# ViennaRNA/RNAcode

Hardware: AMD Instinct MI355X
Metric: alignment-columns x samples scored /sec (higher is better)
Workload: dtype f32; 1 GPU; synthetic MAF 10000 blocks x 120 cols x 6 seqs, n=1000 (BASELINE configs[2]/[3]); exchange=none, fit_exp_mode=fused

## Files before the change

rnacode_amd/csrc/rc_null_kernel.h:

```cpp
#pragma once
#include <hip/hip_runtime.h>

#include <type_traits>
#include <utility>

#include "rc_device.h"
#include "rc_launch.h"

namespace rc {


template <bool SEM> __device__ __forceinline__ float ref_max(float x, float y) {
  if constexpr (SEM) return x > y ? x : y;
  else return fmaxf(x, y);
}
template <bool SEM> __device__ __forceinline__ float ref_max3(float x, float y, float z) { return ref_max<SEM>(ref_max<SEM>(x, y), z); }

template <bool SEM = false>
__device__ __forceinline__ void pair_step(int zc, float sig, float Delta, float Omega, float omega,
                                          float &s0, float &s1, float &s2) {
  if (zc == 0) {
    s0 = s0 + sig;
    s1 = s1 + omega;
    s2 = s2 + omega;
// ... 29 lines not shown

__device__ __forceinline__ void native_scan_rows(const float *rows, int aLo, int aHi, int sites, int s, int f, float tieThr, ScanState &st, int &n,
                                                 DevHss *out, int hssCap, int lane) {
  for (int a = aLo; a < aHi; a++) {
    for (int j0 = a; j0 < sites; j0 += kWave) {
      const int j = j0 + lane;
      const float v = (j < sites) ? rows[static_cast<size_t>(a - aLo) * sites + j] : 0.0f;
      const bool last = (a == sites - 1) && (j == sites - 1);
      unsigned long long m = __ballot((j < sites) && (v > 0.0f || last));
      while (m) {
        const int t = __builtin_ctzll(m);
        m &= m - 1ull;
        const int jj = j0 + t;
        const float vt = __int_as_float(__builtin_amdgcn_readlane(__float_as_int(v), t));
        scan_step(st, vt, a, jj, (a == sites - 1) && (jj == sites - 1), tieThr, [&](const ScanState &e) {
          if (out && lane == 0 && n < hssCap) out[n] = DevHss{s, f, e.ss, e.se, e.cm};
          n++;
        });
      }
    }
  }
}

__device__ __forceinline__ uint32_t codon_flip(uint32_t c) { return ((c & 3u) << 4) | (c & 12u) | ((c >> 4) & 3u); }


template <int K> struct KReg { float s0, s1, s2; int lut; };
template <typename Seq> struct KRegs;
template <int... K> struct KRegs<std::integer_sequence<int, K...>> : KReg<K>... {
  template <int I> __device__ __forceinline__ KReg<I> &at() { return static_cast<KReg<I> &>(*this); }
};
template <int NK, typename F, int... K>
__device__ __forceinline__ void static_for_impl(F &&f, std::integer_sequence<int, K...>) {
  (f(std::integral_constant<int, K>{}), ...);
}
template <int NK, typename F> __device__ __forceinline__ void static_for(F &&f) {
  static_for_impl<NK>(static_cast<F &&>(f), std::make_integer_sequence<int, NK>{});
}

template <int NK, bool EXACT> __device__ __forceinline__ float div_by_nk(float x, float nkf) {
  if constexpr ((NK & (NK - 1)) == 0) {
    return x * (1.0f / static_cast<float>(NK));
  } else if constexpr (EXACT) {
    return x / nkf;
  } else {
    constexpr float y = 1.0f / static_cast<float>(NK);
    const float q0 = x * y;
    const float r = __builtin_fmaf(-static_cast<float>(NK), q0, x);
    return __builtin_fmaf(r, y, q0);
  }
}

struct SampleScan {
  float cm;
  float Q;
  uint32_t se;
  uint32_t len;
};
__device__ __forceinline__ void sample_scan_row_begin(SampleScan &st, float &best, uint32_t a) {
  const bool done = (st.cm > 0.0f) & (st.se < a);
  best = (done & (st.len >= 2u) & (st.cm > best)) ? st.cm : best;
  st.cm = done ? 0.0f : st.cm;
  st.len = done ? 0u : st.len;
  st.Q = static_cast<float>(2u * (st.len + a));
}
__device__ __forceinline__ void sample_scan_step(SampleScan &st, float v, float j2, float negTieThr) {
  const float d = v - st.cm;
  const bool upd = (v > st.cm) | ((v > 0.0f) & (d > negTieThr) & (st.Q <= j2));
  st.cm = upd ? v : st.cm;
  st.Q = upd ? j2 : st.Q;
}
__device__ __forceinline__ void sample_scan_row_end(SampleScan &st, uint32_t a) {
  const uint32_t q = static_cast<uint32_t>(st.Q);
  const bool inrow = (q & 1u) != 0u;
  const uint32_t j = q >> 1;
  st.se = inrow ? j : st.se;
  st.len = inrow ? j - a : st.len;
}
__device__ __forceinline__ void sample_scan_last(const SampleScan &st, float &best) {
  best = ((st.len >= 2u) & (st.cm > best)) ? st.cm : best;
}

struct DeepFetch {};

template <int NK, bool LDSC, bool EXACT, bool DUAL, int MODE = 0>
__device__ __forceinline__ void null_body(const NullArgs &A, const uint8_t *__restrict__ blob,
                                          const DevBlock *__restrict__ dblocks, const int *__restrict__ classBlocks,
                                          const uint32_t *__restrict__ flags, const uint32_t *__restrict__ Ustream, const uint8_t *__restrict__ pairTab,
                                          uint32_t *__restrict__ scratch, float *__restrict__ maxima) {
  constexpr int N = NK + 1;
  constexpr int CPW = 5;
  constexpr int NCW = (NK + CPW - 1) / CPW;
  constexpr bool kTableLookups = !LDSC && !EXACT;
  constexpr int kTableWords = kTableLookups ? NK * kWave : 0;
  constexpr int LB = code_tail_bytes(NK);
  constexpr int PSW = code_pos_words(NK);
  using TailT = std::conditional_t<LB == 1, uint8_t, std::conditional_t<LB == 2, uint16_t, uint32_t>>;
  constexpr int ZW = (NK + 31) / 32;
  using Regs = KRegs<std::make_integer_sequence<int, NK>>;
  static_assert(!DUAL || (!EXACT && NK <= kDualRowsMaxNK), "two rows per pass: fast division, few sequences");
  static_assert(!(LDSC && EXACT), "the EXACT instantiation uses no LDS");
  constexpr bool ROWS = MODE == 1, SIM = MODE == 2;
#ifndef RC_DEEP_FETCH_MAX_NK
#define RC_DEEP_FETCH_MAX_NK 31
#endif
  constexpr bool kDeep = !LDSC && !EXACT && !DUAL && MODE == 0 && NK <= RC_DEEP_FETCH_MAX_NK;
  static_assert(MODE == 0 || (!LDSC && !EXACT && !DUAL), "rows split over workgroups: the one-row kernel that reads its codes from L2");
  extern __shared__ uint32_t lds_codes[];

  const int lane = threadIdx.x;
  unsigned int xcc;
  asm volatile("s_getreg_b32 %0, hwreg(HW_REG_XCC_ID)" : "=s"(xcc));
  const int home = static_cast<int>(xcc & 7u);
  const int rowParts = ROWS ? A.rowParts : 1;
  const int parts = SIM ? A.simParts : A.comboSplit ? 6 * rowParts : 1;
  const int nBlocks = A.nBlocksPtr ? *A.nBlocksPtr : A.nClassBlocks;
  const bool stealing = A.steal != nullptr && !A.comboSplit;
  constexpr int kStealHdr = 16;
  auto claim_part = [&](int slot) -> int {
    unsigned int v = 0;
    if (lane == 0) v = atomicAdd(A.steal + kStealHdr + slot, 1u);
    v = static_cast<unsigned int>(__builtin_amdgcn_readfirstlane(static_cast<int>(v)));
    return (v >= 1u && v <= 6u) ? static_cast<int>(v) - 1 : 6;
  };
  auto steal_word = [&](size_t at) -> unsigned int { return __hip_atomic_load(A.steal + at, __ATOMIC_RELAXED, __HIP_MEMORY_SCOPE_AGENT); };
  int helpCursor = 0;
  bool helping = false;
  for (int qi = 0;;) {
    int bi, grp, onlyCombo = -1, firstCombo = 0, rowPart = 0, itemIndex = 0;
    bool shared = false;
    int slot = static_cast<int>(blockIdx.x);
    if (!helping) {
      if (qi >= 8) {
        if (!stealing) break;
        helping = true;
        continue;
      }
      const int q = (home + qi) & 7;
      const int g0 = A.gLo + ((q - A.gLo) & 7);
      const int gq = g0 < A.gHi ? ((A.gHi - 1 - g0) >> 3) + 1 : 0;
      const int perBlock = gq * parts;
      const int nq = nBlocks * perBlock;
      int t = nq;
      if (nq > 0) {
        if (lane == 0) t = static_cast<int>(atomicAdd((SIM ? A.simCounter : A.workCounter) + q, 1u));
        t = __builtin_amdgcn_readfirstlane(t);
      }
      if (t >= nq) { qi++; continue; }
      bi = classBlocks[t / perBlock];
      if (A.skipMask && (flags[bi] & A.skipMask)) continue;
      const int sub = t % perBlock;
      grp = g0 + 8 * (sub / parts);
      onlyCombo = A.comboSplit ? (sub % parts) / rowParts : -1;
      if constexpr (MODE != 0) { rowPart = SIM ? sub % parts : (sub % parts) % rowParts; itemIndex = (t / perBlock) * (A.gHi - A.gLo) + (grp - A.gLo); }
      if constexpr (MODE != 0) slot = itemIndex;
      if (stealing && nq - t <= static_cast<int>(gridDim.x >> 3) + 16) {
        shared = true;
        if (lane == 0) atomicAdd(A.steal + 1, 1u);
      }
    } else {
      const size_t G = gridDim.x;
      const int np = __builtin_amdgcn_readfirstlane(static_cast<int>(steal_word(0)));
      int victim = -1;
      while (helpCursor < np) {
        const int i = helpCursor + lane;
        const unsigned int ent = i < np ? steal_word(kStealHdr + 3 * G + i) : 0u;
// ... 168 lines not shown
    if constexpr (SIM) continue;
    if (!helping && shared) {
      const size_t G = gridDim.x;
      if (lane == 0) {
        __hip_atomic_store(A.steal + kStealHdr + G + 2 * blockIdx.x, static_cast<unsigned int>(bi), __ATOMIC_RELAXED, __HIP_MEMORY_SCOPE_AGENT);
        __hip_atomic_store(A.steal + kStealHdr + G + 2 * blockIdx.x + 1, static_cast<unsigned int>(grp), __ATOMIC_RELAXED, __HIP_MEMORY_SCOPE_AGENT);
      }
      __builtin_amdgcn_fence(__ATOMIC_RELEASE, "agent");
      __builtin_amdgcn_s_waitcnt(0);
      if (lane == 0) {
        atomicExch(A.steal + kStealHdr + blockIdx.x, 1u);
        const unsigned int idx = atomicAdd(A.steal, 1u);
        __hip_atomic_store(A.steal + kStealHdr + 3 * G + idx, (blockIdx.x + 1u) | (static_cast<unsigned int>(home) << 24), __ATOMIC_RELAXED, __HIP_MEMORY_SCOPE_AGENT);
        atomicSub(A.steal + 1, 1u);
      }
      firstCombo = claim_part(slot);
    }

    float best = -1.0f;
    unsigned long long statCells = 0, statNoPos = 0, statPosLanes = 0, statPristine = 0, statEvent = 0, statTail = 0;
    float omega_v, Delta_v = 0.0f;
    asm volatile("v_mov_b32 %0, %1" : "=v"(omega_v) : "s"(omega));
    float rcpNk_v = 0.0f, negNk_v = 0.0f;
    if constexpr (!EXACT && (NK & (NK - 1)) != 0) {
      asm volatile("v_mov_b32 %0, %1" : "=v"(rcpNk_v) : "s"(1.0f / static_cast<float>(NK)));
      asm volatile("v_mov_b32 %0, %1" : "=v"(negNk_v) : "s"(-static_cast<float>(NK)));
    }
    if constexpr (EXACT) asm volatile("v_mov_b32 %0, %1" : "=v"(Delta_v) : "s"(Delta));
    if (!kProfiling || !(A.debugSkip & 1)) {
      Regs R;
      int curS = -1;
      for (int c = onlyCombo >= 0 ? onlyCombo : firstCombo; c < 6; c = onlyCombo >= 0 ? 6 : (shared ? claim_part(slot) : c + 1)) {
        const int s = c >= 3 ? 1 : 0, f = c - 3 * s;
        if (s != curS) {
          static_for<NK>([&](auto kc) {
            constexpr int k = decltype(kc)::value;
            R.template at<k>().lut = __float_as_int(lut[(s * NK + k) * kLutSize + lane]);
            if constexpr (kTableLookups) lds_codes[k * kWave + lane] = static_cast<uint32_t>(R.template at<k>().lut);
          });
          curS = s;
        }
        const int sites = (L - f) / 3;
        if (sites <= 0) continue;
        const uint32_t *__restrict__ sbase = cod + static_cast<size_t>(s * L1 + 3 + f) * PSW;
        constexpr int kSiteWords = 3 * PSW;
        auto word_at = [&](int j, int x) -> uint32_t {
          const uint32_t *p = sbase + static_cast<size_t>(j) * kSiteWords;
          if (x < NCW - 1) return p[x * kWave + lane];
          return static_cast<uint32_t>(reinterpret_cast<const TailT *>(p + (NCW - 1) * kWave)[lane]);
        };
        const unsigned long long *__restrict__ zbase = zw + static_cast<size_t>(s * L1 + 3 + f) * ZW;
        const unsigned long long *__restrict__ zany = zmask + static_cast<size_t>(s * 3 + f) * zmWords;
        int jc = sites;
        constexpr int kCacheSiteBytes = PSW * 4;
        if constexpr (LDSC) {
          for (int idx = 0; idx < sites * NCW; idx++) lds_codes[idx * kWave + lane] = word_at(idx / NCW, idx % NCW);
          __builtin_amdgcn_s_waitcnt(0);
        } else if constexpr (!EXACT) {
          jc = sites - (A.cacheSites < sites ? A.cacheSites : sites);
          for (int j = jc; j < sites; j++) {
            uint32_t *dst = lds_codes + kTableWords + (j - jc) * PSW;
#pragma unroll
            for (int x = 0; x < NCW - 1; x++) dst[x * kWave + lane] = word_at(j, x);
            reinterpret_cast<TailT *>(dst + (NCW - 1) * kWave)[lane] = static_cast<TailT>(word_at(j, NCW - 1));
          }
          __builtin_amdgcn_s_waitcnt(0);
        }
        const uint32_t ldsBase = static_cast<uint32_t>(reinterpret_cast<uintptr_t>(lds_codes + kTableWords));
        const uint32_t ldsLane = ldsBase + static_cast<uint32_t>(lane) * 4u;
        const uint32_t ldsTail = ldsBase + (NCW - 1) * kWave * 4u + static_cast<uint32_t>(lane) * LB;
        const uint32_t laneOff = static_cast<uint32_t>(lane) * 4u, laneTail = static_cast<uint32_t>(lane) * LB;
        [[maybe_unused]] const uint8_t *ldsBytesAll = reinterpret_cast<const uint8_t *>(lds_codes + kTableWords) - ldsBase;
        auto fetch_staged = [&](uint32_t (&w)[NCW], int j) {
          const uint32_t at = ldsLane + static_cast<uint32_t>(j) * (NCW * kWave * 4u);
#pragma unroll
          for (int x = 0; x < NCW; x++) {
#ifdef RC_PLAIN_FETCH
            w[x] = *reinterpret_cast<const uint32_t *>(ldsBytesAll + at + x * kWave * 4);
#else
            asm volatile("ds_read_b32 %0, %1 offset:%2" : "=v"(w[x]) : "v"(at), "n"(x * kWave * 4));
#endif
          }
        };
        auto fetch_cached = [&](uint32_t (&w)[NCW], int j) {
          const uint32_t off = static_cast<uint32_t>(j - jc) * kCacheSiteBytes;
#ifdef RC_PLAIN_FETCH
          if constexpr (NCW > 1) {
#pragma unroll
            for (int x = 0; x < NCW - 1; x++) w[x] = *reinterpret_cast<const uint32_t *>(ldsBytesAll + ldsLane + off + x * kWave * 4);
          }
          w[NCW - 1] = static_cast<uint32_t>(*reinterpret_cast<const TailT *>(ldsBytesAll + ldsTail + off));
#else
          if constexpr (NCW > 1) {
            const uint32_t at = ldsLane + off;
#pragma unroll
            for (int x = 0; x < NCW - 1; x++) asm volatile("ds_read_b32 %0, %1 offset:%2" : "=v"(w[x]) : "v"(at), "n"(x * kWave * 4));
          }
          const uint32_t att = ldsTail + off;
          if constexpr (LB == 1) asm volatile("ds_read_u8 %0, %1" : "=v"(w[NCW - 1]) : "v"(att));
          else if constexpr (LB == 2) asm volatile("ds_read_u16 %0, %1" : "=v"(w[NCW - 1]) : "v"(att));
          else asm volatile("ds_read_b32 %0, %1" : "=v"(w[NCW - 1]) : "v"(att));
#endif
        };
        auto fetch_global = [&](uint32_t (&w)[NCW], const uint32_t *p) {
          const uint32_t lo = laneOff + 0u, lt = laneTail + 0u;
#ifdef RC_PLAIN_FETCH
          const uint8_t *pb = reinterpret_cast<const uint8_t *>(p);
#pragma unroll
          for (int x = 0; x < NCW - 1; x++) w[x] = *reinterpret_cast<const uint32_t *>(pb + lo + x * kWave * 4);
          w[NCW - 1] = static_cast<uint32_t>(*reinterpret_cast<const TailT *>(pb + lt + (NCW - 1) * kWave * 4));
          return;
#endif
#pragma unroll
          for (int x = 0; x < NCW - 1; x++) asm volatile("global_load_dword %0, %1, %2 offset:%3" : "=v"(w[x]) : "v"(lo), "s"(p), "n"(x * kWave * 4));
          if constexpr (LB == 1) asm volatile("global_load_ubyte %0, %1, %2 offset:%3" : "=v"(w[NCW - 1]) : "v"(lt), "s"(p), "n"((NCW - 1) * kWave * 4));
          else if constexpr (LB == 2) asm volatile("global_load_ushort %0, %1, %2 offset:%3" : "=v"(w[NCW - 1]) : "v"(lt), "s"(p), "n"((NCW - 1) * kWave * 4));
          else asm volatile("global_load_dword %0, %1, %2 offset:%3" : "=v"(w[NCW - 1]) : "v"(lt), "s"(p), "n"((NCW - 1) * kWave * 4));
        };
        auto load_words = [&](int j, uint32_t (&w)[NCW]) {
          if constexpr (LDSC) {
#pragma unroll
            for (int x = 0; x < NCW; x++) w[x] = lds_codes[(j * NCW + x) * kWave + lane];
          } else if constexpr (!EXACT) {
            if (j >= jc) {
              fetch_cached(w, j);
            } else {
              const uint32_t *p = sbase + static_cast<size_t>(j) * kSiteWords;
              asm volatile("s_nop 4" : "+s"(p));
              fetch_global(w, p);
            }
#pragma unroll
            for (int x = 0; x < NCW; x++) asm volatile("s_waitcnt vmcnt(0) lgkmcnt(0)" : "+v"(w[x]));
          } else {
#pragma unroll
            for (int x = 0; x < NCW; x++) w[x] = word_at(j, x);
          }
        };
        auto lookup = [&](uint32_t (&w)[NCW], float (&sig)[NK], int jn, auto scalarLoadsNearby, auto kind) {
          if constexpr (LDSC) {
#pragma unroll
            for (int x = 0; x < NCW; x++) asm volatile("s_waitcnt lgkmcnt(0)" : "+v"(w[x]));
          }
          const uint32_t *pnext = sbase + static_cast<size_t>(jn) * kSiteWords;
          if constexpr (!LDSC && !EXACT) asm volatile("" : "+s"(pnext));
          static_for<NK>([&](auto kc) {
            constexpr int k = decltype(kc)::value;
            constexpr int t = k % CPW;
            constexpr int kYounger = std::is_same_v<std::decay_t<decltype(kind)>, DeepFetch> ? NCW : 0;
            if constexpr (!LDSC && !EXACT && t == 0) asm volatile("s_waitcnt vmcnt(%1)" : "+v"(w[k / CPW]) : "n"(NCW - 1 - k / CPW + kYounger));
            uint32_t addr;
            if constexpr (t == 0) addr = w[k / CPW]; else addr = w[k / CPW] >> (6 * t);
            float got;
            if constexpr (kTableLookups) {
              uint32_t at;
              asm volatile("v_and_b32 %0, 0xfc, %1" : "=v"(at) : "v"(addr));
              asm volatile("ds_read_b32 %0, %1 offset:%2" : "=v"(got) : "v"(at), "n"(k * kWave * 4));
            } else {
              const int lutv = R.template at<k>().lut;
              asm volatile("ds_bpermute_b32 %0, %1, %2" : "=v"(got) : "v"(addr), "v"(lutv));
            }
            sig[k] = got;
          });
          auto wait_lookups = [&](auto leave) {
            constexpr int k0 = (NCW - 1) * CPW;
            constexpr int cnt = NK - k0;
            constexpr int left = (decltype(leave)::value > 0 && !decltype(scalarLoadsNearby)::value) ? decltype(leave)::value : 0;
            if constexpr (cnt == 1) asm volatile("s_waitcnt lgkmcnt(%1)" : "+v"(sig[k0]) : "n"(left));
            else if constexpr (cnt == 2) asm volatile("s_waitcnt lgkmcnt(%2)" : "+v"(sig[k0]), "+v"(sig[k0 + 1]) : "n"(left));
            else if constexpr (cnt == 3) asm volatile("s_waitcnt lgkmcnt(%3)" : "+v"(sig[k0]), "+v"(sig[k0 + 1]), "+v"(sig[k0 + 2]) : "n"(left));
            else if constexpr (cnt == 4)
              asm volatile("s_waitcnt lgkmcnt(%4)" : "+v"(sig[k0]), "+v"(sig[k0 + 1]), "+v"(sig[k0 + 2]), "+v"(sig[k0 + 3]) : "n"(left));
            else
              asm volatile("s_waitcnt lgkmcnt(%5)" : "+v"(sig[k0]), "+v"(sig[k0 + 1]), "+v"(sig[k0 + 2]), "+v"(sig[k0 + 3]), "+v"(sig[k0 + 4]) : "n"(left));
            static_for<NK>([&](auto kc) {
              constexpr int k = decltype(kc)::value;
              if constexpr (k < k0) {
                float b = sig[k];
                asm volatile("" : "+v"(b), "+v"(sig[k0]));
                sig[k] = b;
              }
            });
          };
          if constexpr (LDSC) {
            fetch_staged(w, jn);
            wait_lookups(std::integral_constant<int, NCW>{});
          } else if constexpr (!EXACT) {
            if constexpr (std::is_same_v<std::decay_t<decltype(kind)>, DeepFetch>) fetch_global(w, pnext);
            else if (jn >= jc) fetch_cached(w, jn);
            else fetch_global(w, pnext);
            wait_lookups(std::integral_constant<int, 0>{});
          } else {
            wait_lookups(std::integral_constant<int, 0>{});
          }
        };
        auto finish = [&](float sum) -> float {
          if constexpr (kProfiling) {
            const unsigned long long pos = __ballot(sum > 0.0f);
            statCells++; statNoPos += (pos == 0ull); statPosLanes += __builtin_popcountll(pos);
          }
          if constexpr (EXACT) {
            const float top = (sum > Delta_v) ? sum : Delta_v;
            return div_by_nk<NK, EXACT>(top, nkf);
          } else {
            if constexpr ((NK & (NK - 1)) == 0) return div_by_nk<NK, EXACT>(sum, nkf);
            else {
              const float q0 = sum * rcpNk_v;
              const float r = __builtin_fmaf(negNk_v, q0, sum);
              return __builtin_fmaf(r, rcpNk_v, q0);
            }
          }
        };
        auto fast_cell = [&](uint32_t (&w)[NCW], int jn, auto kind) -> float {
          float sig[NK];
          lookup(w, sig, jn, std::false_type{}, kind);
          float sum = 0.0f;
          static_for<NK>([&](auto kc) {
            constexpr int k = decltype(kc)::value;
            auto &r = R.template at<k>();
            r.s0 = r.s0 + sig[k];
            r.s1 = r.s1 + omega_v;
            r.s2 = r.s2 + omega_v;
            const float m = fmaxf(fmaxf(r.s0, r.s1), r.s2);
            sum = (k == 0) ? m : sum + m;
          });
          return finish(sum);
        };
        auto pristine_cell = [&](uint32_t (&w)[NCW], float &wv, int jn, auto kind) -> float {
          float sig[NK];
          lookup(w, sig, jn, std::false_type{}, kind);
          wv = wv + omega_v;
          float sum = 0.0f;
          static_for<NK>([&](auto kc) {
            constexpr int k = decltype(kc)::value;
            auto &r = R.template at<k>();
            r.s0 = r.s0 + sig[k];
            const float m = fmaxf(r.s0, wv);
            sum = (k == 0) ? m : sum + m;
          });
          return finish(sum);
        };
        auto tail_cell = [&](uint32_t (&w)[NCW], int jn, auto kind) -> float {
          float sig[NK];
          lookup(w, sig, jn, std::false_type{}, kind);
          float sum = 0.0f;
          static_for<NK>([&](auto kc) {
            constexpr int k = decltype(kc)::value;
            auto &r = R.template at<k>();
            r.s0 = r.s0 + sig[k];
            r.s1 = r.s1 + omega_v;
            const float m = fmaxf(r.s0, r.s1);
            sum = (k == 0) ? m : sum + m;
          });
          return finish(sum);
        };
        auto event_cell = [&](uint32_t (&w)[NCW], int j, int jn, auto kind) -> float {
          float sig[NK];
          lookup(w, sig, jn, std::true_type{}, kind);
          unsigned long long z[ZW];
#pragma unroll
          for (int x = 0; x < ZW; x++) z[x] = zbase[static_cast<size_t>(3 * j) * ZW + x];
          float sum = 0.0f;
          static_for<NK>([&](auto kc) {
            constexpr int k = decltype(kc)::value;
            auto &r = R.template at<k>();
            pair_step(static_cast<int>((z[k >> 5] >> (2 * (k & 31))) & 3ull), sig[k], Delta, Omega, omega, r.s0, r.s1, r.s2);
            const float m = fmaxf(fmaxf(r.s0, r.s1), r.s2);
            sum = (k == 0) ? m : sum + m;
          });
          return finish(sum);
        };
        auto nan_cell = [&](uint32_t (&w)[NCW], int j, int jn, auto kind) -> float {
          float sig[NK];
          lookup(w, sig, jn, std::true_type{}, kind);
          unsigned long long z[ZW];
#pragma unroll
          for (int x = 0; x < ZW; x++) z[x] = zbase[static_cast<size_t>(3 * j) * ZW + x];
          float sum = 0.0f;
          static_for<NK>([&](auto kc) {
            constexpr int k = decltype(kc)::value;
            auto &r = R.template at<k>();
            pair_step<true>(static_cast<int>((z[k >> 5] >> (2 * (k & 31))) & 3ull), sig[k], Delta, Omega, omega, r.s0, r.s1, r.s2);
            const float m = ref_max3<true>(r.s0, r.s1, r.s2);
            sum = (k == 0) ? m : sum + m;
          });
          return finish(sum);
        };
        auto next_event = [&](int j, int end) -> int {
          while (j < end) {
            const unsigned long long mword = zany[j >> 6] >> (j & 63);
            if (mword) { const int e = j + __builtin_ctzll(mword); return e < end ? e : end; }
            j = (j | 63) + 1;
          }
          return end;
        };
        SampleScan st{0.0f, 0.0f, 0u, 0u};
        float two_v;
        asm volatile("v_mov_b32 %0, 2.0" : "=v"(two_v));
        const float negTie = -A.tieThr;
        if constexpr (DUAL) {
          typedef float RowBuf __attribute__((ext_vector_type(32)));
          constexpr int kBuf = 32;
          RowBuf buf = {};
          Regs RB;
          auto pristine2 = [&](uint32_t (&w)[NCW], float &wvA, float &wvB, int jn, float &vB, auto kd) -> float {
            float sig[NK];
            lookup(w, sig, jn, std::false_type{}, kd);
            wvA = wvA + omega_v;
            wvB = wvB + omega_v;
            float sumA = 0.0f, sumB = 0.0f;
            static_for<NK>([&](auto kc) {
              constexpr int k = decltype(kc)::value;
              auto &ra = R.template at<k>();
              auto &rb = RB.template at<k>();
              ra.s0 = ra.s0 + sig[k];
              const float ma = fmaxf(ra.s0, wvA);
              sumA = (k == 0) ? ma : sumA + ma;
              rb.s0 = rb.s0 + sig[k];
              const float mb = fmaxf(rb.s0, wvB);
              sumB = (k == 0) ? mb : sumB + mb;
            });
            vB = finish(sumB);
            return finish(sumA);
          };
          auto fast2 = [&](uint32_t (&w)[NCW], int jn, float &vB, auto kd) -> float {
            float sig[NK];
            lookup(w, sig, jn, std::false_type{}, kd);
            float sumA = 0.0f, sumB = 0.0f;
            static_for<NK>([&](auto kc) {
              constexpr int k = decltype(kc)::value;
              auto &ra = R.template at<k>();
              auto &rb = RB.template at<k>();
              ra.s0 = ra.s0 + sig[k];
              ra.s1 = ra.s1 + omega_v;
              ra.s2 = ra.s2 + omega_v;
              const float ma = fmaxf(fmaxf(ra.s0, ra.s1), ra.s2);
              sumA = (k == 0) ? ma : sumA + ma;
              rb.s0 = rb.s0 + sig[k];
              rb.s1 = rb.s1 + omega_v;
              rb.s2 = rb.s2 + omega_v;
              const float mb = fmaxf(fmaxf(rb.s0, rb.s1), rb.s2);
              sumB = (k == 0) ? mb : sumB + mb;
            });
            vB = finish(sumB);
            return finish(sumA);
          };
          auto tail2 = [&](uint32_t (&w)[NCW], int jn, float &vB, auto kd) -> float {
            float sig[NK];
            lookup(w, sig, jn, std::false_type{}, kd);
            float sumA = 0.0f, sumB = 0.0f;
            static_for<NK>([&](auto kc) {
              constexpr int k = decltype(kc)::value;
              auto &ra = R.template at<k>();
              auto &rb = RB.template at<k>();
              ra.s0 = ra.s0 + sig[k];
              ra.s1 = ra.s1 + omega_v;
              const float ma = fmaxf(ra.s0, ra.s1);
              sumA = (k == 0) ? ma : sumA + ma;
              rb.s0 = rb.s0 + sig[k];
              rb.s1 = rb.s1 + omega_v;
              const float mb = fmaxf(rb.s0, rb.s1);
              sumB = (k == 0) ? mb : sumB + mb;
            });
            vB = finish(sumB);
            return finish(sumA);
          };
          auto event2 = [&](uint32_t (&w)[NCW], int j, int jn, float &vB) -> float {
            float sig[NK];
            lookup(w, sig, jn, std::true_type{}, std::true_type{});
            unsigned long long z[ZW];
#pragma unroll
            for (int x = 0; x < ZW; x++) z[x] = zbase[static_cast<size_t>(3 * j) * ZW + x];
            float sumA = 0.0f, sumB = 0.0f;
            static_for<NK>([&](auto kc) {
              constexpr int k = decltype(kc)::value;
              auto &ra = R.template at<k>();
              auto &rb = RB.template at<k>();
              const int zc = static_cast<int>((z[k >> 5] >> (2 * (k & 31))) & 3ull);
              pair_step(zc, sig[k], Delta, Omega, omega, ra.s0, ra.s1, ra.s2);
              const float ma = fmaxf(fmaxf(ra.s0, ra.s1), ra.s2);
              sumA = (k == 0) ? ma : sumA + ma;
              pair_step(zc, sig[k], Delta, Omega, omega, rb.s0, rb.s1, rb.s2);
              const float mb = fmaxf(fmaxf(rb.s0, rb.s1), rb.s2);
              sumB = (k == 0) ? mb : sumB + mb;
            });
            vB = finish(sumB);
            return finish(sumA);
          };
          int a = 0;
          int pendRow = -1, pendExtra = 0, pendN = 0;
          while (a < sites || pendRow >= 0) {
            if (pendRow < 0 && a + 2 < sites && !((zany[a >> 6] >> (a & 63)) & 1ull)) {
              sample_scan_row_begin(st, best, static_cast<uint32_t>(a));
              static_for<NK>([&](auto kc) {
                constexpr int k = decltype(kc)::value;
                auto &r = R.template at<k>();
                r.s0 = r.s1 = r.s2 = 0.0f;
                auto &rb = RB.template at<k>();
                rb.s0 = rb.s1 = rb.s2 = 0.0f;
              });
              uint32_t wcur[NCW];
              load_words(a, wcur);
              int j = a;
              float j2f = static_cast<float>(2 * a + 1);
              float wvA = 0.0f, wvB = 0.0f;
              asm volatile("v_mov_b32 %0, 0" : "=v"(wvA));
              asm volatile("v_mov_b32 %0, 0" : "=v"(wvB));
              {
                const float v = pristine_cell(wcur, wvA, a + 1, std::true_type{});
                sample_scan_step(st, v, j2f, negTie);
                asm volatile("v_add_f32 %0, %1, %0" : "+v"(j2f) : "v"(two_v));
                j = a + 1;
              }
              const int extra = (sites - 1 - a > kBuf) ? sites - 1 - a - kBuf : 0;
              const int b0 = a + 1 + extra;
              auto keep = [&](float vB, int jj) {
                const int idx = jj > b0 ? jj - b0 : 0;
                buf[idx] = vB;
              };
              auto pair_cell = [&](uint32_t (&w)[NCW], int jj, int jn, auto kd, auto &&fn) {
                float vB;
                const float v = fn(w, jn, vB, kd);
                sample_scan_step(st, v, j2f, negTie);
                keep(vB, jj);
                const float two_c = two_v;
                asm volatile("v_add_f32 %0, %1, %0" : "+v"(j2f) : "v"(two_c));
              };
              auto dspan = [&](int e, auto &&fn) {
                if constexpr (!LDSC && !EXACT && MODE == 0) {
                  const int lim = e < jc - 2 ? e : jc - 2;
                  if (lim - j >= 4) {
                    uint32_t wB[NCW];
                    {
                      const uint32_t *p = sbase + static_cast<size_t>(j + 1) * kSiteWords;
                      asm volatile("s_nop 4" : "+s"(p));
                      fetch_global(wB, p);
                    }
                    for (; j + 2 <= lim; j += 2) {
                      pair_cell(wcur, j, j + 2, DeepFetch{}, fn);
                      pair_cell(wB, j + 1, j + 3, DeepFetch{}, fn);
                    }
#pragma unroll
                    for (int x = 0; x < NCW; x++) asm volatile("s_waitcnt vmcnt(0)" : "+v"(wB[x]));
                  }
                }
                for (; j < e; j++) pair_cell(wcur, j, j + 1 < sites ? j + 1 : j, std::true_type{}, fn);
              };
              {
                dspan(next_event(j, sites), [&](uint32_t (&w)[NCW], int jn, float &vB, auto kd) { return pristine2(w, wvA, wvB, jn, vB, kd); });
                static_for<NK>([&](auto kc) {
                  constexpr int k = decltype(kc)::value;
                  auto &r = R.template at<k>();
                  r.s1 = r.s2 = wvA;
                  auto &rb = RB.template at<k>();
                  rb.s1 = rb.s2 = wvB;
                });
              }
              while (j < sites) {
                if ((zany[j >> 6] >> (j & 63)) & 1ull) {
                  const int jev = j;
                  pair_cell(wcur, j, j + 1 < sites ? j + 1 : j, std::true_type{}, [&](uint32_t (&w)[NCW], int jn, float &vB, auto) { return event2(w, jev, jn, vB); });
                  j++;
                }
                const int e = next_event(j, sites);
                if (e == sites) {
                  static_for<NK>([&](auto kc) {
                    constexpr int k = decltype(kc)::value;
                    auto &r = R.template at<k>();
                    r.s1 = fmaxf(r.s1, r.s2);
                    auto &rb = RB.template at<k>();
                    rb.s1 = fmaxf(rb.s1, rb.s2);
                  });
                  dspan(e, [&](uint32_t (&w)[NCW], int jn, float &vB, auto kd) { return tail2(w, jn, vB, kd); });
                }
                dspan(e, [&](uint32_t (&w)[NCW], int jn, float &vB, auto kd) { return fast2(w, jn, vB, kd); });
              }
#pragma unroll
              for (int x = 0; x < NCW; x++) asm volatile("s_waitcnt lgkmcnt(0)" : "+v"(wcur[x]));
              sample_scan_row_end(st, static_cast<uint32_t>(a));
              pendRow = a + 1; pendExtra = extra; pendN = sites - b0;
              a += 2;
            } else {
              const bool pend = pendRow >= 0;
              const int row = pend ? pendRow : a;
              const int jend = pend ? row + pendExtra : ((row == sites - 1) ? sites - 1 : sites);
              float j2f = static_cast<float>(2 * row + 1);
                sample_scan_row_begin(st, best, static_cast<uint32_t>(row));
                static_for<NK>([&](auto kc) {
                  constexpr int k = decltype(kc)::value;
                  auto &r = R.template at<k>();
                  r.s0 = r.s1 = r.s2 = 0.0f;
                });
                uint32_t wcur[NCW];
                load_words(row, wcur);
                int j = row;
                {
                  const int e = next_event(j, jend);
                  float wv = 0.0f;
                  asm volatile("v_mov_b32 %0, 0" : "=v"(wv));
                  for (; j < e; j++) {
                    const int jn = j + 1 < sites ? j + 1 : j;
                    uint32_t wnext[NCW];
                    if constexpr (EXACT) load_words(jn, wnext);
                    if constexpr (kProfiling) statPristine++;
                    const float v = pristine_cell(wcur, wv, jn, std::true_type{});
                    sample_scan_step(st, v, j2f, negTie);
                    asm volatile("v_add_f32 %0, %1, %0" : "+v"(j2f) : "v"(two_v));
                    if constexpr (EXACT) {
      #pragma unroll
                      for (int x = 0; x < NCW; x++) wcur[x] = wnext[x];
                    }
                  }
                  static_for<NK>([&](auto kc) {
                    constexpr int k = decltype(kc)::value;
                    auto &r = R.template at<k>();
                    r.s1 = r.s2 = wv;
                  });
                }
                while (j < jend) {
                  if ((zany[j >> 6] >> (j & 63)) & 1ull) {
                    const int jn = j + 1 < sites ? j + 1 : j;
                    uint32_t wnext[NCW];
                    if constexpr (EXACT) load_words(jn, wnext);
                    if constexpr (kProfiling) statEvent++;
                    const float v = event_cell(wcur, j, jn, std::true_type{});
                    sample_scan_step(st, v, j2f, negTie);
                    asm volatile("v_add_f32 %0, %1, %0" : "+v"(j2f) : "v"(two_v));
                    if constexpr (EXACT) {
      #pragma unroll
                      for (int x = 0; x < NCW; x++) wcur[x] = wnext[x];
                    }
                    j++;
                  }
                  const int e = next_event(j, jend);
                  if (e == jend) {
                    static_for<NK>([&](auto kc) {
                      constexpr int k = decltype(kc)::value;
                      auto &r = R.template at<k>();
                      r.s1 = fmaxf(r.s1, r.s2);
                    });
                    for (; j < e; j++) {
                      const int jn = j + 1 < sites ? j + 1 : j;
                      uint32_t wnext[NCW];
                      if constexpr (EXACT) load_words(jn, wnext);
                      if constexpr (kProfiling) statTail++;
                      const float v = tail_cell(wcur, jn, std::true_type{});
                      sample_scan_step(st, v, j2f, negTie);
                      asm volatile("v_add_f32 %0, %1, %0" : "+v"(j2f) : "v"(two_v));
                      if constexpr (EXACT) {
      #pragma unroll
                        for (int x = 0; x < NCW; x++) wcur[x] = wnext[x];
                      }
                    }
                  }
                  for (; j < e; j++) {
                    const int jn = j + 1 < sites ? j + 1 : j;
                    uint32_t wnext[NCW];
                    if constexpr (EXACT) load_words(jn, wnext);
// ... 84 lines not shown
                    asm volatile("s_nop 4" : "+s"(p));
                    fetch_global(wB, p);
                  }
                  for (; j + 2 <= lim; j += 2) {
                    take(cell(wcur, j + 2, DeepFetch{}));
                    take(cell(wB, j + 3, DeepFetch{}));
                  }
#pragma unroll
                  for (int x = 0; x < NCW; x++) asm volatile("s_waitcnt vmcnt(0)" : "+v"(wB[x]));
                }
              }
              for (; j < e; j++) one(cell);
            };
            if constexpr (EXACT) {
              if (nanSem)
                for (; j < jend; j++) {
                  const int jj = j;
                  one([&](uint32_t (&w)[NCW], int jn, auto kd) { return nan_cell(w, jj, jn, kd); });
                }
            }
            {
              const int e = next_event(j, jend);
              float wv = 0.0f;
              asm volatile("v_mov_b32 %0, 0" : "=v"(wv));
              span(e, [&](uint32_t (&w)[NCW], int jn, auto kd) {
                if constexpr (kProfiling) statPristine++;
                return pristine_cell(w, wv, jn, kd);
              });
              static_for<NK>([&](auto kc) {
                constexpr int k = decltype(kc)::value;
                auto &r = R.template at<k>();
                r.s1 = r.s2 = wv;
              });
            }
            while (j < jend) {
              if ((zany[j >> 6] >> (j & 63)) & 1ull) {
                if constexpr (kProfiling) statEvent++;
                const int jj = j;
                one([&](uint32_t (&w)[NCW], int jn, auto kd) { return event_cell(w, jj, jn, kd); });
                j++;
              }
              const int e = next_event(j, jend);
              if (e == jend) {
                static_for<NK>([&](auto kc) {
                  constexpr int k = decltype(kc)::value;
                  auto &r = R.template at<k>();
                  r.s1 = fmaxf(r.s1, r.s2);
                });
                span(e, [&](uint32_t (&w)[NCW], int jn, auto kd) {
                  if constexpr (kProfiling) statTail++;
                  return tail_cell(w, jn, kd);
                });
              }
              span(e, [&](uint32_t (&w)[NCW], int jn, auto kd) { return fast_cell(w, jn, kd); });
            }
            if constexpr (!EXACT) {
#pragma unroll
              for (int x = 0; x < NCW; x++) {
                if constexpr (LDSC) asm volatile("s_waitcnt lgkmcnt(0)" : "+v"(wcur[x]));
                else asm volatile("s_waitcnt vmcnt(0) lgkmcnt(0)" : "+v"(wcur[x]));
              }
            }
            if constexpr (ROWS) { if (a == sites - 1) sdst += kWave; }
            else sample_scan_row_end(st, static_cast<uint32_t>(a));
          }
        }
        if constexpr (!ROWS) sample_scan_last(st, best);
      }
    }
    if constexpr (kProfiling) {
      if (A.cellStats && lane == 0) {
        atomicAdd(A.cellStats, statCells); atomicAdd(A.cellStats + 1, statNoPos); atomicAdd(A.cellStats + 2, statPosLanes);
        atomicAdd(A.cellStats + 3, statPristine); atomicAdd(A.cellStats + 4, statEvent); atomicAdd(A.cellStats + 5, statTail);
      }
    }
    if (!ROWS && sidx < A.sampleN) {
      float *dst = maxima + static_cast<size_t>(db->out_index) * A.sampleN + sidx;
      if (A.comboSplit || shared) { if (best > -1.0f) atomicMax(reinterpret_cast<int *>(dst), __float_as_int(best)); }
      else *dst = best;
    }
  }
}

constexpr int null_min_waves(int NK, bool EXACT, bool DUAL, int MODE) { return (EXACT || DUAL || MODE != 0) ? 1 : NK == 6 ? 6 : (NK == 9 || NK == 10) ? 5 : (NK >= 16 && NK <= 21) ? 4 : (NK >= 24 && NK <= 29) ? 3 : 1; }
template <int NK, bool LDSC, bool EXACT, bool DUAL = false, int MODE = 0>
__global__ __launch_bounds__(64) __attribute__((amdgpu_waves_per_eu(null_min_waves(NK, EXACT, DUAL, MODE))))
void k_null(NullArgs A, const uint8_t *__restrict__ blob,
                                             const DevBlock *__restrict__ dblocks, const int *__restrict__ classBlocks,
                                             const uint32_t *__restrict__ flags, const uint32_t *__restrict__ Ustream, const uint8_t *__restrict__ pairTab,
                                             uint32_t *__restrict__ scratch, float *__restrict__ maxima) {
  null_body<NK, LDSC, EXACT, DUAL, MODE>(A, blob, dblocks, classBlocks, flags, Ustream, pairTab, scratch, maxima);
}

constexpr int hi_occ_waves(int NK) { return (NK >= 6 && NK <= 8) ? 6 : (NK >= 10 && NK <= 12) ? 5 : 0; }
template <int NK>
__global__ __launch_bounds__(64) __attribute__((amdgpu_waves_per_eu(hi_occ_waves(NK) ? hi_occ_waves(NK) : 1)))
void k_null_occ(NullArgs A, const uint8_t *__restrict__ blob, const DevBlock *__restrict__ dblocks, const int *__restrict__ classBlocks,
                const uint32_t *__restrict__ flags, const uint32_t *__restrict__ Ustream, const uint8_t *__restrict__ pairTab,
                uint32_t *__restrict__ scratch, float *__restrict__ maxima) {
  null_body<NK, false, false, false>(A, blob, dblocks, classBlocks, flags, Ustream, pairTab, scratch, maxima);
}


template <int NK> constexpr size_t phase_a_lds() { return NK < kFastRows ? static_cast<size_t>(kPhaseALds) : static_cast<size_t>(2 * (NK + 1)) * 64 + 64 * 64; }

template <int NK>
inline int null_occupancy_one(size_t ldsBytes) {
  int nb = 0;
  hipError_t e = ldsBytes ? hipOccupancyMaxActiveBlocksPerMultiprocessor(&nb, k_null<NK, true, false>, 64, ldsBytes)
                          : hipOccupancyMaxActiveBlocksPerMultiprocessor(&nb, k_null<NK, false, false>, 64, phase_a_lds<NK>());
  if (e != hipSuccess) return 0;
  return nb;
}
template <int NK>
inline int null_occupancy_plain_one(size_t dynLds, int hiOcc) {
  int nb = 0;
  hipError_t e;
  if (hiOcc == 2) {
    if constexpr (NK >= 3 && NK <= kDualRowsMaxNK) e = hipOccupancyMaxActiveBlocksPerMultiprocessor(&nb, k_null<NK, false, false, true>, 64, dynLds);
    else return 0;
  } else if (hiOcc) {
    if constexpr (hi_occ_waves(NK) != 0) e = hipOccupancyMaxActiveBlocksPerMultiprocessor(&nb, k_null_occ<NK>, 64, dynLds);
    else return 0;
  } else e = hipOccupancyMaxActiveBlocksPerMultiprocessor(&nb, k_null<NK, false, false>, 64, dynLds);
  if (e != hipSuccess) return 0;
  return nb;
}

template <int NK>
inline void launch_null_one(const NullArgs &a, int grid, size_t ldsBytes, bool exact, hipStream_t stream) {
  if (exact) {
    hipLaunchKernelGGL((k_null<NK, false, true>), dim3(grid), dim3(64), 0, stream, a, a.blob, a.dblocks,
                       a.classBlocks, a.flags, a.U, a.pair, a.scratch, a.maxima);
  } else if (ldsBytes) {
    if constexpr (NK <= kDualRowsMaxNK) {
      if (a.dual && ldsBytes <= 48 * 1024) {
        hipLaunchKernelGGL((k_null<NK, true, false, true>), dim3(grid), dim3(64), ldsBytes, stream, a, a.blob, a.dblocks,
                           a.classBlocks, a.flags, a.U, a.pair, a.scratch, a.maxima);
        return;
      }
    }
    if (ldsBytes > 48 * 1024)
      (void)hipFuncSetAttribute(reinterpret_cast<const void *>(k_null<NK, true, false>),
                                hipFuncAttributeMaxDynamicSharedMemorySize, static_cast<int>(ldsBytes));
    hipLaunchKernelGGL((k_null<NK, true, false>), dim3(grid), dim3(64), ldsBytes, stream, a, a.blob, a.dblocks,
                       a.classBlocks, a.flags, a.U, a.pair, a.scratch, a.maxima);
  } else {
    const size_t dyn = a.plainLds ? static_cast<size_t>(a.plainLds) : phase_a_lds<NK>();
    if constexpr (NK < kFastRows) {
      if (a.rowParts > 1) {
        hipLaunchKernelGGL((k_null<NK, false, false, false, 2>), dim3(a.simGrid), dim3(64), phase_a_lds<NK>(), stream, a, a.blob, a.dblocks,
                           a.classBlocks, a.flags, a.U, a.pair, a.scratch, a.maxima);
        hipLaunchKernelGGL((k_null<NK, false, false, false, 1>), dim3(grid), dim3(64), dyn, stream, a, a.blob, a.dblocks,
                           a.classBlocks, a.flags, a.U, a.pair, a.scratch, a.maxima);
        return;
      }
    }
    if constexpr (NK >= 3 && NK <= kDualRowsMaxNK) {
      if (a.hiOcc == 2) {
        hipLaunchKernelGGL((k_null<NK, false, false, true>), dim3(grid), dim3(64), dyn, stream, a, a.blob, a.dblocks,
                           a.classBlocks, a.flags, a.U, a.pair, a.scratch, a.maxima);
        return;
      }
    }
    if constexpr (hi_occ_waves(NK) != 0) {
      if (a.hiOcc) {
        hipLaunchKernelGGL((k_null_occ<NK>), dim3(grid), dim3(64), dyn, stream, a, a.blob, a.dblocks,
// ... 63 lines not shown
```

Baseline: 27.49 billion alignment-columns*samples/s.

## Unroll dual-row LDS-staged scan in groups of four with immediate-offset reads

In the dual-row path with LDS-staged codes, the inner site loop now runs in groups of four sites. It computes one base LDS address per group and issues ds_read with compile-time offsets for each site, then writes the four second-row values to the row buffer between scheduling barriers. The DUAL instantiation also raises its waves-per-EU hint to 4, which may force fewer registers and cause spills. The aim is to cut per-site address arithmetic and loop overhead and to let reads from several sites overlap.

```diff
diff --git a/rnacode_amd/csrc/rc_null_kernel.h b/rnacode_amd/csrc/rc_null_kernel.h
--- a/rnacode_amd/csrc/rc_null_kernel.h
+++ b/rnacode_amd/csrc/rc_null_kernel.h
@@ -135,6 +135,12 @@
 }
 
 struct DeepFetch {};
+template <int OFF> struct StagedSite { uint32_t at; };
+template <typename T> struct IsStagedSite : std::false_type {};
+template <int OFF> struct IsStagedSite<StagedSite<OFF>> : std::true_type {};
+template <int OFF> constexpr int staged_off(StagedSite<OFF>) { return OFF; }
+__device__ __forceinline__ int site_index(int j) { return j; }
+template <int OFF> __device__ __forceinline__ int site_index(StagedSite<OFF>) { return 0; }
 
 template <int NK, bool LDSC, bool EXACT, bool DUAL, int MODE = 0>
 __device__ __forceinline__ void null_body(const NullArgs &A, const uint8_t *__restrict__ blob,
@@ -469,6 +475,19 @@
 #endif
           }
         };
+        auto fetch_staged_at = [&](uint32_t (&w)[NCW], auto site) {
+          constexpr int off = staged_off(decltype(site){});
+          static_assert(off + NCW * kWave * 4 <= 65536, "ds_read offset: 16 bits");
+          const uint32_t at = site.at;
+#pragma unroll
+          for (int x = 0; x < NCW; x++) {
+#ifdef RC_PLAIN_FETCH
+            w[x] = *reinterpret_cast<const uint32_t *>(ldsBytesAll + at + off + x * kWave * 4);
+#else
+            asm volatile("ds_read_b32 %0, %1 offset:%2" : "=v"(w[x]) : "v"(at), "n"(off + x * kWave * 4));
+#endif
+          }
+        };
         auto fetch_cached = [&](uint32_t (&w)[NCW], int j) {
           const uint32_t off = static_cast<uint32_t>(j - jc) * kCacheSiteBytes;
 #ifdef RC_PLAIN_FETCH
@@ -523,12 +542,12 @@
             for (int x = 0; x < NCW; x++) w[x] = word_at(j, x);
           }
         };
-        auto lookup = [&](uint32_t (&w)[NCW], float (&sig)[NK], int jn, auto scalarLoadsNearby, auto kind) {
+        auto lookup = [&](uint32_t (&w)[NCW], float (&sig)[NK], auto jn, auto scalarLoadsNearby, auto kind) {
           if constexpr (LDSC) {
 #pragma unroll
             for (int x = 0; x < NCW; x++) asm volatile("s_waitcnt lgkmcnt(0)" : "+v"(w[x]));
           }
-          const uint32_t *pnext = sbase + static_cast<size_t>(jn) * kSiteWords;
+          const uint32_t *pnext = sbase + static_cast<size_t>(site_index(jn)) * kSiteWords;
           if constexpr (!LDSC && !EXACT) asm volatile("" : "+s"(pnext));
           static_for<NK>([&](auto kc) {
             constexpr int k = decltype(kc)::value;
@@ -569,7 +588,8 @@
             });
           };
           if constexpr (LDSC) {
-            fetch_staged(w, jn);
+            if constexpr (IsStagedSite<std::decay_t<decltype(jn)>>::value) fetch_staged_at(w, jn);
+            else fetch_staged(w, jn);
             wait_lookups(std::integral_constant<int, NCW>{});
           } else if constexpr (!EXACT) {
             if constexpr (std::is_same_v<std::decay_t<decltype(kind)>, DeepFetch>) fetch_global(w, pnext);
@@ -687,9 +707,10 @@
         if constexpr (DUAL) {
           typedef float RowBuf __attribute__((ext_vector_type(32)));
           constexpr int kBuf = 32;
+          constexpr int kGroup = 4;
           RowBuf buf = {};
           Regs RB;
-          auto pristine2 = [&](uint32_t (&w)[NCW], float &wvA, float &wvB, int jn, float &vB, auto kd) -> float {
+          auto pristine2 = [&](uint32_t (&w)[NCW], float &wvA, float &wvB, auto jn, float &vB, auto kd) -> float {
             float sig[NK];
             lookup(w, sig, jn, std::false_type{}, kd);
             wvA = wvA + omega_v;
@@ -709,7 +730,7 @@
             vB = finish(sumB);
             return finish(sumA);
           };
-          auto fast2 = [&](uint32_t (&w)[NCW], int jn, float &vB, auto kd) -> float {
+          auto fast2 = [&](uint32_t (&w)[NCW], auto jn, float &vB, auto kd) -> float {
             float sig[NK];
             lookup(w, sig, jn, std::false_type{}, kd);
             float sumA = 0.0f, sumB = 0.0f;
@@ -731,7 +752,7 @@
             vB = finish(sumB);
             return finish(sumA);
           };
-          auto tail2 = [&](uint32_t (&w)[NCW], int jn, float &vB, auto kd) -> float {
+          auto tail2 = [&](uint32_t (&w)[NCW], auto jn, float &vB, auto kd) -> float {
             float sig[NK];
             lookup(w, sig, jn, std::false_type{}, kd);
             float sumA = 0.0f, sumB = 0.0f;
@@ -830,10 +851,40 @@
                     for (int x = 0; x < NCW; x++) asm volatile("s_waitcnt vmcnt(0)" : "+v"(wB[x]));
                   }
                 }
+                if constexpr (LDSC) {
+                  for (const int pe = e < b0 ? e : b0; j < pe; j++) {
+                    float vB;
+                    const float v = fn(wcur, j + 1, vB, std::true_type{});
+                    sample_scan_step(st, v, j2f, negTie);
+                    const float two_c = two_v;
+                    asm volatile("v_add_f32 %0, %1, %0" : "+v"(j2f) : "v"(two_c));
+                  }
+                  const int ge = e < sites - 1 ? e : sites - 1;
+                  for (; j + kGroup <= ge; j += kGroup) {
+                    const uint32_t at = ldsLane + static_cast<uint32_t>(j + 1) * (NCW * kWave * 4u);
+                    float vB[kGroup];
+                    static_for<kGroup>([&](auto uc) {
+                      constexpr int u = decltype(uc)::value;
+                      const float v = fn(wcur, StagedSite<u * NCW * kWave * 4>{at}, vB[u], std::true_type{});
+                      sample_scan_step(st, v, j2f, negTie);
+                      const float two_c = two_v;
+                      asm volatile("v_add_f32 %0, %1, %0" : "+v"(j2f) : "v"(two_c));
+                    });
+                    int idxRaw = j - b0;
+                    asm volatile("" : "+s"(idxRaw));
+                    const int idx = idxRaw & (kBuf - 1);
+                    __builtin_amdgcn_sched_barrier(0);
+                    static_for<kGroup>([&](auto uc) {
+                      constexpr int u = decltype(uc)::value;
+                      buf[idx + u] = vB[u];
+                    });
+                    __builtin_amdgcn_sched_barrier(0);
+                  }
+                }
                 for (; j < e; j++) pair_cell(wcur, j, j + 1 < sites ? j + 1 : j, std::true_type{}, fn);
               };
               {
-                dspan(next_event(j, sites), [&](uint32_t (&w)[NCW], int jn, float &vB, auto kd) { return pristine2(w, wvA, wvB, jn, vB, kd); });
+                dspan(next_event(j, sites), [&](uint32_t (&w)[NCW], auto jn, float &vB, auto kd) { return pristine2(w, wvA, wvB, jn, vB, kd); });
                 static_for<NK>([&](auto kc) {
                   constexpr int k = decltype(kc)::value;
                   auto &r = R.template at<k>();
@@ -857,9 +908,9 @@
                     auto &rb = RB.template at<k>();
                     rb.s1 = fmaxf(rb.s1, rb.s2);
                   });
-                  dspan(e, [&](uint32_t (&w)[NCW], int jn, float &vB, auto kd) { return tail2(w, jn, vB, kd); });
+                  dspan(e, [&](uint32_t (&w)[NCW], auto jn, float &vB, auto kd) { return tail2(w, jn, vB, kd); });
                 }
-                dspan(e, [&](uint32_t (&w)[NCW], int jn, float &vB, auto kd) { return fast2(w, jn, vB, kd); });
+                dspan(e, [&](uint32_t (&w)[NCW], auto jn, float &vB, auto kd) { return fast2(w, jn, vB, kd); });
               }
 #pragma unroll
               for (int x = 0; x < NCW; x++) asm volatile("s_waitcnt lgkmcnt(0)" : "+v"(wcur[x]));
@@ -1110,7 +1161,7 @@
   }
 }
 
-constexpr int null_min_waves(int NK, bool EXACT, bool DUAL, int MODE) { return (EXACT || DUAL || MODE != 0) ? 1 : NK == 6 ? 6 : (NK == 9 || NK == 10) ? 5 : (NK >= 16 && NK <= 21) ? 4 : (NK >= 24 && NK <= 29) ? 3 : 1; }
+constexpr int null_min_waves(int NK, bool EXACT, bool DUAL, int MODE) { return DUAL ? 4 : (EXACT || MODE != 0) ? 1 : NK == 6 ? 6 : (NK == 9 || NK == 10) ? 5 : (NK >= 16 && NK <= 21) ? 4 : (NK >= 24 && NK <= 29) ? 3 : 1; }
 template <int NK, bool LDSC, bool EXACT, bool DUAL = false, int MODE = 0>
 __global__ __launch_bounds__(64) __attribute__((amdgpu_waves_per_eu(null_min_waves(NK, EXACT, DUAL, MODE))))
 void k_null(NullArgs A, const uint8_t *__restrict__ blob,
```

Measured after the change: 28.10 billion alignment-columns*samples/s (median of 6 runs). 2.2% higher.
